# thawro/pytorch-human-pose

Hardware: AMD Instinct MI355X
Metric: images/sec (fwd+decode) HigherHRNet-W32 512px (higher is better)
Workload: dtype bf16; 1 GPU; HigherHRNet-W32 inference bf16, batch 32 @ 512x512 per GPU (conv fwd on N(0,1) images + AE decode on constructed maps, 10 people/image, det_thr 0.05, tag_thr 0.5, adjust+refine); global_batch=32, parallelism=image-sharded replicas x1, no data-path collective

## Files before the change

### include/hhrnet.h

```cpp
#ifndef HHRNET_H
#define HHRNET_H
#include <stdint.h>

#ifdef __cplusplus
extern "C" {
#endif

#define HH_ABI_VERSION 3
#define HH_DTYPE_BF16 1
#define HH_DTYPE_FP8 2
#define HH_DTYPE_F16 3

typedef struct hh_net hh_net;
typedef struct hh_decoder hh_decoder;

int hh_abi_version(void);
const char *hh_last_error(void);

hh_net *hh_create(int num_kpts, int C, int dtype);
void hh_destroy(hh_net *net);

hh_net *hh_create_classifier(int C, int num_classes, int dtype);
int hh_forward_classifier(hh_net *net, const float *images, int B, int H, int W, float *logits, void *stream);

int hh_num_params(const hh_net *net);
const char *hh_param_name(const hh_net *net, int index);
int hh_param_shape(const hh_net *net, int index, int64_t shape[4]);

int hh_load_weights(hh_net *net, const char *name, const float *host, const int64_t *shape, int ndim);
int hh_finalize(hh_net *net);

int hh_calibrate(hh_net *net, const float *images, int B, int H, int W, int rounds, void *stream);

int hh_e4m3_encode(const float *x, int64_t n, unsigned char *out);
int hh_e4m3_decode(const unsigned char *x, int64_t n, float *out);

int hh_reserve(hh_net *net, int B, int H, int W);
int64_t hh_workspace_bytes(const hh_net *net);

int hh_forward(hh_net *net, const float *images, int B, int H, int W, float *init_heatmaps, float *deconv_heatmaps,
               int use_graph, void *stream);

int hh_set_multi_lane(hh_net *net, int enable);

int hh_debug_check_plan(const hh_net *net);

double hh_forward_flops(const hh_net *net, int B, int H, int W);

int hh_profile_enable(hh_net *net, int enable);
int hh_profile_count(const hh_net *net);
int hh_profile_get(hh_net *net, int index, int *cfg, double *flops, double *bytes, float *ms, float *kernel_ms, const char **layer);
int hh_profile_clock(hh_net *net, int index, double *ghz);
int hh_conv_config(int cfg, int out[7]);
int hh_conv_config_double_buffered(int cfg);

int hh_debug_conv_bench(int cfg, int B, int Hin, int Win, int cin, int cout, int with_res, int relu, int iters,
                        float *ms_per_launch, unsigned long long *stamps16, int ref_cfg, float *max_diff);

int hh_debug_bb_bench(int B, int H, int W, int iters, float *ms_per_launch, unsigned long long *stamps64);
int hh_debug_bb_compare(int B, int H, int W, int iters, float *max_diff, float *ms_classic, float *ms_pc);

int hh_debug_bb_cover(int B, int H, int W, int tall, int num_cus, int64_t counts[4]);

int hh_set_taps(hh_net *net, int enable);
int hh_num_taps(const hh_net *net);
const char *hh_tap_name(const hh_net *net, int index);
int hh_tap_shape(const hh_net *net, int index, int64_t shape[4]);
int hh_tap_read(hh_net *net, int index, float *host_nchw);

int hh_preprocess_u8(const unsigned char *image_hwc, int h, int w, const double dst_to_src[6], float *out_nchw, int H, int W,
                     const float mean[3], const float stdv[3], void *stream);

typedef struct hh_image_desc {
    long long offset;
    int h, w;
    double dst_to_src[6];
} hh_image_desc;
int hh_preprocess_u8_batch(const unsigned char *images_base, const hh_image_desc *descs_dev, int n, float *out_nchw, int H, int W,
                           const float mean[3], const float stdv[3], void *stream);

int hh_flip_images(const float *images, float *out, int B, int C, int H, int W, void *stream);
int hh_flip_merge(float *hm, int64_t hm_bstride, const float *hm_flipped, int64_t hmf_bstride, const float *tags_flipped,
                  int64_t tf_bstride, float *tags_out, int64_t to_bstride, const int32_t *perm_host, int B, int K,
                  int h, int w, void *stream);

hh_decoder *hh_decoder_create(int num_kpts, int max_people, double det_thr, double tag_thr);
void hh_decoder_destroy(hh_decoder *dec);
int hh_decoder_reserve(hh_decoder *dec, int B, int H, int W, int E);
int hh_decoder_set_exact_topk(hh_decoder *dec, int enable);

#define HH_DECODE_FALLBACK 1
#define HH_DECODE_SOLVER_GUARD 2
int hh_decode(hh_decoder *dec, const float *hm_q, int64_t hm_q_bstride, const float *hm_h, int64_t hm_h_bstride,
              const float *const *tags_q, const int64_t *tags_bstride, int E, int B, int hq, int wq, int adjust,
              int refine, float *joints, float *scores, int32_t *num_people, int32_t *flags, void *stream);

int hh_parse(hh_decoder *dec, const float *hm_full, const float *tags_full, int E, int B, int H, int W, int adjust,
             int refine, float *joints, float *scores, int32_t *num_people, int32_t *flags, void *stream);
// ... 309 lines not shown
```

### pytorch-human-pose_amd/csrc/capi.cpp

```cpp
#include <cmath>
#include <cstdint>
#include <cstring>
#include <string>
#include <vector>

#include "../../include/hhrnet.h"
#include "engine.h"
#include "optim_math.h"
#include "grad_stats_math.h"
#include "ema_math.h"
#include "render_math.h"
#include "panel_math.h"
#include "coco_eval_math.h"
#include "crowd_mask_math.h"
#include "track_math.h"

const char *hh_get_error();
int hh_tap_read_impl(hh_net *n, int index, float *host);

extern "C" {

int hh_abi_version(void) { return HH_ABI_VERSION; }
const char *hh_last_error(void) { return hh_get_error(); }

// ... 70 lines not shown
int hh_e4m3_encode(const float *x, int64_t n, unsigned char *out)
{
    for (int64_t i = 0; i < n; ++i) out[i] = hh_f32_to_e4m3(x[i]);
    return 0;
}
int hh_e4m3_decode(const unsigned char *x, int64_t n, float *out)
{
    for (int64_t i = 0; i < n; ++i) out[i] = hh_e4m3_to_f32(x[i]);
    return 0;
}
int hh_finalize(hh_net *net) { return net->finalize(); }
int hh_calibrate(hh_net *net, const float *images, int B, int H, int W, int rounds, void *stream)
{
    if (!images || B <= 0 || H <= 0 || W <= 0 || H % 32 || W % 32) { hh_set_error("hh_calibrate: need images [B,3,H,W] with H, W multiples of 32"); return 1; }
    return net->calibrate(images, B, H, W, rounds > 0 ? rounds : 2, (hipStream_t)stream);
}
int hh_reserve(hh_net *net, int B, int H, int W) { return net->reserve(B, H, W); }
int64_t hh_workspace_bytes(const hh_net *net) { return net->ws_bytes; }

int hh_forward(hh_net *net, const float *images, int B, int H, int W, float *init_heatmaps, float *deconv_heatmaps,
               int use_graph, void *stream)
{
    if (net->kind != 0) { hh_set_error("hh_forward: classifier handle, use hh_forward_classifier"); return 1; }
    if (!images || !init_heatmaps || !deconv_heatmaps) { hh_set_error("hh_forward: null buffer"); return 1; }
    if (B <= 0 || H <= 0 || W <= 0 || H % 32 || W % 32) { hh_set_error("hh_forward: H and W must be positive multiples of 32"); return 1; }
    return net->forward(images, B, H, W, init_heatmaps, deconv_heatmaps, use_graph, (hipStream_t)stream);
}
double hh_forward_flops(const hh_net *net, int B, int H, int W) { return net->flops(B, H, W); }

int hh_set_multi_lane(hh_net *net, int enable)
{
    net->multi_lane = enable != 0;
    for (auto &g : net->graphs) hipGraphExecDestroy(g.exec);
    net->graphs.clear();
    return 0;
}
int hh_set_taps(hh_net *net, int enable) { net->taps_enabled = enable != 0; return 0; }
int hh_num_taps(const hh_net *net) { return (int)net->taps.size(); }
const char *hh_tap_name(const hh_net *net, int i) { return (i >= 0 && i < (int)net->taps.size()) ? net->taps[i].name.c_str() : nullptr; }
int hh_tap_shape(const hh_net *net, int i, int64_t shape[4])
{
    if (i < 0 || i >= (int)net->taps.size()) return 1;
    const TensorDesc &d = net->tensors[net->taps[i].tensor];
    shape[0] = net->lastB; shape[1] = net->taps[i].C; shape[2] = net->lastH >> d.shift; shape[3] = net->lastW >> d.shift;
    return 0;
}
int hh_tap_read(hh_net *net, int index, float *host_nchw) { return hh_tap_read_impl(net, index, host_nchw); }

int hh_debug_check_plan(const hh_net *net)
{
    std::string why;
    if (net->check_plan(&why)) { hh_set_error("schedule hazard: " + why); return 1; }
    return 0;
}

int hh_profile_enable(hh_net *net, int enable) { net->prof_enabled = enable != 0; net->prof_clk = enable == 2; net->prof_used = 0; return 0; }
int hh_profile_count(const hh_net *net) { return (int)net->prof_used; }
int hh_profile_get(hh_net *net, int i, int *cfg, double *flops, double *bytes, float *ms, float *kernel_ms, const char **layer)
{
    if (i < 0 || i >= (int)net->prof_used) { hh_set_error("hh_profile_get: index out of range"); return 1; }
    const ProfRecord &r = net->prof[i];
    HH_CHECK_HIP(hipEventSynchronize(r.e1));
    HH_CHECK_HIP(hipEventElapsedTime(ms, r.e0, r.e1));
    *cfg = r.cfg; *flops = r.flops; *bytes = r.bytes;
    *layer = net->layers[net->ops[r.op].layer].conv.c_str();
    *kernel_ms = -1.f;
    if (r.slot >= 0 && net->prof_clk && net->d_clk && net->clk_khz > 0) {
        unsigned long long t[2];
        HH_CHECK_HIP(hipMemcpy(t, net->d_clk + 4 * r.slot, 16, hipMemcpyDeviceToHost));
        if (t[1] > t[0]) *kernel_ms = (float)((double)(t[1] - t[0]) / net->clk_khz);
    }
    return 0;
}
int hh_profile_clock(hh_net *net, int i, double *ghz)
{
    if (i < 0 || i >= (int)net->prof_used) { hh_set_error("hh_profile_clock: index out of range"); return 1; }
    const ProfRecord &r = net->prof[i];
    *ghz = 0.0;
    if (r.slot >= 0 && net->prof_clk && net->d_clk && net->clk_khz > 0) {
        unsigned long long t[2];
        HH_CHECK_HIP(hipEventSynchronize(r.e1));
        HH_CHECK_HIP(hipMemcpy(t, net->d_clk + 4 * r.slot + 2, 16, hipMemcpyDeviceToHost));
        if (t[1]) *ghz = (double)t[0] / (double)t[1] * net->clk_khz * 1e-6;
    }
    return 0;
}
int hh_conv_config(int cfg, int out[7])
{
    if (cfg >= 1000 && cfg - 1000 < conv_fp8_num_configs()) {
        const Fp8ConvConfig &c = conv_fp8_config(cfg - 1000);
        out[0] = c.KS; out[1] = c.S; out[2] = c.KC; out[3] = c.NT; out[4] = 1; out[5] = c.PT; out[6] = c.TW;
        return 0;
    }
    if (cfg < 0 || cfg >= conv_num_configs()) return 1;
    const ConvConfig &c = conv_config(cfg);
    out[0] = c.KS; out[1] = c.S; out[2] = c.KC; out[3] = c.NT; out[4] = c.WC; out[5] = c.PT; out[6] = c.TW;
    return 0;
}

int hh_conv_config_double_buffered(int cfg)
{
    if (cfg >= 1000 && cfg - 1000 < conv_fp8_num_configs()) return 0;
    if (cfg < 0 || cfg >= conv_num_configs()) return -1;
    return conv_config(cfg).DB;
}

// ... 1562 lines not shown
```

### pytorch-human-pose_amd/csrc/engine.cpp

```cpp
#include "engine.h"
#include "f16_host.h"

#include <cmath>
#include <cstdlib>
#include <cstring>

static thread_local std::string g_err;
LaunchProbe &hh_launch_probe()
{
    static thread_local LaunchProbe p;
    return p;
}
void hh_set_error(const std::string &msg) { g_err = msg; }
const char *hh_get_error() { return g_err.c_str(); }

PlanSwitches PlanSwitches::from_env()
{
    auto on = [](const char *name) { const char *v = getenv(name); return v && *v && strcmp(v, "0"); };
    auto is = [](const char *name, const char *val) { const char *v = getenv(name); return v && !strcmp(v, val); };
    PlanSwitches s;
    s.bb32_tile = is("HH_BB32", "tile");
    s.no_bb64 = on("HH_NO_BB64");
    s.no_stem_fused = on("HH_NO_STEM_FUSED");
    s.no_junc_pair = on("HH_NO_JUNC_PAIR");
    s.full_join = on("HH_FULL_JOIN");
    s.no_fusion_merge = on("HH_NO_FUSION_MERGE");
    s.no_fused_upsum = on("HH_NO_FUSED_UPSUM");
    s.poison_ws = on("HH_POISON_WS");
    s.poison_lds = on("HH_POISON_LDS");
    s.no_head_fold = on("HH_NO_HEAD_FOLD");
    s.no_conv_db = on("HH_NO_CONV_DB");
    s.no_final_fuse = on("HH_NO_FINAL_FUSE");
    s.keep_waits = on("HH_KEEP_WAITS");
    s.event_system_fence = on("HH_EVENT_SYSTEM_FENCE");
    s.bb_tall = on("HH_NO_BB_TALL") ? 0 : is("HH_BB_TALL", "always") ? 2 : 1;
    s.fp8_trunk8 = is("HH_FP8_TRUNK", "e4m3");
    s.fp8_heads8 = is("HH_FP8_HEADS", "e4m3");
    return s;
}

static inline int round_up(int v, int m) { return (v + m - 1) / m * m; }

static inline bf16_raw f2bf(float f)
{
    uint32_t u;
    memcpy(&u, &f, 4);
    if ((u & 0x7fffffffu) > 0x7f800000u) return (bf16_raw)((u >> 16) | 0x40);
    u += 0x7fffu + ((u >> 16) & 1u);
    return (bf16_raw)(u >> 16);
}
static inline float bf2f(bf16_raw h)
{
    uint32_t u = (uint32_t)h << 16;
    float f;
    memcpy(&f, &u, 4);
    return f;
}
bf16_raw hh_net::cvt16(float f) const { return act() ? hh_f32_to_f16(f) : f2bf(f); }
float hh_net::widen16(bf16_raw v) const { return act() ? hh_f16_to_f32(v) : bf2f(v); }
int hh_net::check_packed(const std::vector<bf16_raw> &packed, const std::string &param_name) const
{
    if (!act()) return 0;
    for (bf16_raw v : packed)
        if (hh_f16_is_inf(v)) {
            hh_set_error("hh_finalize: " + param_name + ": a BatchNorm-folded weight exceeds the fp16 range (+-65504); use a bf16 handle for this checkpoint");
            return 1;
        }
    return 0;
}

int hh_net::add_param(const std::string &name, std::vector<int64_t> shape, bool counter)
{
    ParamSlot p;
    p.name = name;
    p.shape = std::move(shape);
// ... 114 lines not shown
                p_conv(up + ".conv2", mid, mid, 3); p_bn(up + ".bn2", mid);
                p_conv(up + ".conv3", mid, outs[i], 1); p_bn(up + ".bn3", outs[i]);
                if (w[i] != outs[i]) { p_conv(up + ".downsample.0", w[i], outs[i], 1); p_bn(up + ".downsample.1", outs[i]); }
            }
            for (int i = 0; i < 3; ++i) {
                const std::string dpn = hp + ".downsample_blocks." + std::to_string(i);
                p_conv(dpn + ".0", outs[i], outs[i + 1], 3, true); p_bn(dpn + ".1", outs[i + 1]);
            }
            p_conv(hp + ".final_conv.0", 1024, 2048, 1, true); p_bn(hp + ".final_conv.1", 2048);
            n.add_param(hp + ".classifier.weight", {n.num_classes, 2048});
            n.add_param(hp + ".classifier.bias", {n.num_classes});
            return;
        }
        p_conv("init_heatmaps_head", C, 2 * K, 1, true);
        const std::string dp = "deconv_layers.0";
        n.add_param(dp + ".deconv.0.weight", {C + 2 * K, C, 4, 4});
        p_bn(dp + ".deconv.1", C);
        for (int r = 0; r < 4; ++r) {
            const std::string rp = dp + ".resid_blocks." + std::to_string(r);
            p_conv(rp + ".conv1", C, C, 3); p_bn(rp + ".bn1", C);
            p_conv(rp + ".conv2", C, C, 3); p_bn(rp + ".bn2", C);
        }
        p_conv(dp + ".final_layer", C, K, 1, true);
    }

    int T(int C, int shift, bool zero = false)
    {
        TensorDesc t;
        t.C = C; t.shift = shift; t.zero_init = zero;
        n.tensors.push_back(t);
        return (int)n.tensors.size() - 1;
    }
    int L(const std::string &conv, const std::string &bn, int cin, int cout, int ks, int stride, const std::string &bias = "")
    {
        ConvLayer l;
        l.conv = conv; l.bn = bn; l.bias = bias; l.cin = cin; l.cout = cout; l.ks = ks; l.stride = stride;
        n.layers.push_back(l);
        return (int)n.layers.size() - 1;
    }
    Op &conv(int layer, int in, int out, int relu, int res = -1)
    {
        Op o;
        o.kind = OP_CONV; o.layer = layer; o.in = in; o.out = out; o.relu = relu; o.res = res; o.lane = lane;
        n.ops.push_back(o);
        return n.ops.back();
    }
    Op &cb(const std::string &p, const char *c, const char *b, int cin, int cout, int ks, int stride, int in, int out,
           int relu, int res = -1)
    {
        return conv(L(p + "." + c, p + "." + b, cin, cout, ks, stride), in, out, relu, res);
    }
    void basic_blocks(const std::string &prefix, int C, int x, int m, int nscales = 0, int branch = 0)
    {
        for (int u = 0; u < 4; ++u) {
            const std::string up = prefix + "." + std::to_string(u);
            const bool fused_fp8 = n.dtype == 2 && bb_fp8_supported(C) && branch == 0;
            if (((C == 32 || (C == 64 && !n.sw.no_bb64)) && n.is16()) || fused_fp8) {
                Op o;
                o.kind = OP_BB;
                o.layer = L(up + ".conv1", up + ".bn1", C, C, 3, 1);
                o.layer2 = L(up + ".conv2", up + ".bn2", C, C, 3, 1);
                o.in = (u & 1) ? m : x;
                o.out = (u & 1) ? x : m;
                o.lane = lane;
                o.siblings = nscales > 1;
                n.ops.push_back(o);
            } else {
                cb(up, "conv1", "bn1", C, C, 3, 1, x, m, 1);
                cb(up, "conv2", "bn2", C, C, 3, 1, m, x, 1, x);
            }
        }
    }
    void tap(const std::string &name, int tensor, int C, int coff = 0)
    {
        TapInfo t;
        t.name = name; t.tensor = tensor; t.coff = coff; t.C = C;
        n.taps.push_back(t);
        Op o;
        o.kind = OP_TAP; o.tap = (int)n.taps.size() - 1; o.lane = lane;
        n.ops.push_back(o);
    }

    void build_plan()
    {
        const int C = n.C, K = n.K;
        const int w[4] = {C, 2 * C, 4 * C, 8 * C};
        const std::string bb = "backbone";
        const bool stem_fused = n.is16() && !n.sw.no_stem_fused;
        const int S1 = stem_fused ? -1 : T(64, 1), X = T(64, 2);
        {
            Op o;
            o.kind = OP_STEM; o.layer = L(bb + ".conv1", bb + ".bn1", 3, 64, 3, 2); o.out = stem_fused ? X : S1;
            n.layers[o.layer].stem = true;
            if (stem_fused) {
                o.layer2 = L(bb + ".conv2", bb + ".bn2", 64, 64, 3, 2);
                n.layers[o.layer2].stem2 = true;
            }
            n.ops.push_back(o);
        }
        if (!stem_fused) conv(L(bb + ".conv2", bb + ".bn2", 64, 64, 3, 2), S1, X, 1);

        const bool jpair = n.is16() && !n.sw.no_junc_pair;
        const int t1 = T(64, 2), t2 = T(64, 2), t2b = jpair ? T(64, 2) : t2, Y = T(256, 2);
        auto unit = [&](int u) { return bb + ".stages.0.blocks.0.scales_blocks.0." + std::to_string(u); };
        cb(unit(0), "conv1", "bn1", 64, 64, 1, 1, X, t1, 1);
        const int DS = n.dtype == 2 ? T(256, 2) : -1;
        int prev_conv3 = -1, ds_layer = -1;
        for (int u = 0; u < 4; ++u) {
            const std::string up = unit(u);
            const int t2u = (u & 1) ? t2b : t2, t2p = (u & 1) ? t2 : t2b;
// ... 283 lines not shown
                        for (int j = 0; j < 8; ++j, ++o) {
                            const int co = cg * COUT_T + ci_o, ci = ch * KC + c8 * 8 + j;
                            if (co >= cout || ci >= cin) continue;
                            float v;
                            if (transposed) v = W[(((size_t)ci * cout + co) * 4 + ky) * 4 + kx];
                            else v = W[(((size_t)co * cin + ci) * ks + ky) * ks + kx];
                            packed[o] = act_dtype ? hh_f32_to_f16(v * scale[co]) : f2bf(v * scale[co]);
                        }
            }
}

int hh_family_pick(int ks, int stride, int cin_pad, int coutp, int *KC, int *NT)
{
    if (ks == 3 && stride == 1) *KC = (cin_pad % 32 == 0) ? 32 : 16;
    else if (ks == 1) *KC = (cin_pad % 32 == 0) ? 32 : 16;
    else *KC = 16;
    *NT = (coutp % 64 == 0) ? 2 : 1;
    for (int i = 0; i < conv_num_configs(); ++i) {
        const ConvConfig &c = conv_config(i);
        if (c.KS == ks && c.S == stride && c.KC == *KC && c.NT == *NT && !c.DB) return 0;
    }
    return 1;
}

float hh_net::bn_fold(const std::string &bn, int co, const float *cb, float *shift) const
{
    const float g = param(bn + ".weight")[co], bta = param(bn + ".bias")[co];
    const float mu = param(bn + ".running_mean")[co], var = param(bn + ".running_var")[co];
    const float sc = g / std::sqrt(var + 1e-5f);
    *shift = cb ? bta + (*cb - mu) * sc : bta - mu * sc;
    return sc;
}

void hh_net::fold_layer(const ConvLayer &l, int coutp, std::vector<float> &scale, std::vector<float> &shift) const
{
    scale.assign(coutp, 0.f);
    shift.assign(coutp, 0.f);
    for (int co = 0; co < l.cout; ++co) {
        const float cb = l.bias.empty() ? 0.f : param(l.bias)[co];
        if (l.bn.empty()) { scale[co] = 1.f; shift[co] = cb; }
        else scale[co] = bn_fold(l.bn, co, &cb, &shift[co]);
    }
}

int hh_net::finalize()
{
    for (auto &p : params)
        if (!p.loaded && !p.counter) { hh_set_error("hh_finalize: parameter never loaded: " + p.name); return 1; }
    HH_CHECK_HIP(conv_init());
    HH_CHECK_HIP(bb_fused_init());
    HH_CHECK_HIP(stem_fused_init());
    HH_CHECK_HIP(bbpc_init());
    HH_CHECK_HIP(bb64_fused_init());
    HH_CHECK_HIP(junction_init());
    if (dtype == 2 && kind != 0) { hh_set_error("hh_finalize: the fp8 path covers HigherHRNet only"); return 1; }
    {
        int dev = 0;
        hipDeviceProp_t prop;
        HH_CHECK_HIP(hipGetDevice(&dev));
        HH_CHECK_HIP(hipGetDeviceProperties(&prop, dev));
        num_cus = prop.multiProcessorCount;
    }
    for (auto &l : layers) {
        if (l.stem) {
            const std::vector<float> &W = param(l.conv + ".weight");
            std::vector<bf16_raw> packed(64 * 32, 0);
            std::vector<float> shift(64);
            for (int co = 0; co < 64; ++co) {
                const float sc = bn_fold(l.bn, co, nullptr, &shift[co]);
                for (int t = 0; t < 27; ++t) {
                    const int kk = t / 16, hh = (t % 16) / 8, j = t % 8;
                    packed[((((co / 32) * 2 + kk) * 2 + hh) * 32 + co % 32) * 8 + j] = cvt16(W[(size_t)co * 27 + t] * sc);
                }
            }
            if (check_packed(packed, l.conv + ".weight")) return 1;
            if (hh_upload(&l.d_w, packed.data(), packed.size() * 2) || hh_upload(&l.d_bias, shift.data(), 64 * 4)) return 1;
            continue;
        }
        if (dtype == 2 && !l.hi) continue;
        const int cin_pad0 = round_up(l.cin, 16), coutp = round_up(l.cout, 32);
        if (l.stem2) { l.KC = 64; l.NT = 2; }
        else if (hh_family_pick(l.ks, l.stride, cin_pad0, coutp, &l.KC, &l.NT)) {
            hh_set_error("no kernel family for conv " + l.conv);
            return 1;
        }
        l.db = !sw.no_conv_db && !l.stem2 && l.ks == 3 && l.stride == 1 && !l.transposed && l.mconv.empty() && l.cin >= 128 &&
               l.cin % 16 == 0 && coutp % 64 == 0;
        if (l.db) { l.KC = 16; l.NT = 2; }
        l.cin_pad = round_up(l.cin, l.KC);
        const int COUT_T = 32 * l.NT;
        l.ncg = coutp / COUT_T;
        if (!l.mconv.empty()) {
            std::vector<float> Wm((size_t)l.cout * l.cin * 9, 0.f), one(coutp, 1.f), shift(coutp, 0.f);
            int c0 = 0;
            for (size_t m = 0; m < l.mconv.size(); ++m) {
                if (l.mcin[m] % l.KC) { hh_set_error("merged fusion conv: input width not a multiple of the chunk size"); return 1; }
                const std::vector<float> &Wj = param(l.mconv[m] + ".weight");
                for (int co = 0; co < l.cout; ++co) {
                    float sh;
                    const float sc = bn_fold(l.mbn[m], co, nullptr, &sh);
                    shift[co] += sh;
                    for (int ci = 0; ci < l.mcin[m]; ++ci)
                        for (int t = 0; t < 9; ++t) Wm[((size_t)co * l.cin + c0 + ci) * 9 + t] = Wj[((size_t)co * l.mcin[m] + ci) * 9 + t] * sc;
                    if (act())
                        for (int i = 0; i < l.mcin[m] * 9; ++i)
                            if (hh_f16_is_inf(hh_f32_to_f16(Wj[(size_t)co * l.mcin[m] * 9 + i] * sc))) return check_packed({0x7c00}, l.mconv[m] + ".weight");
// ... 360 lines not shown
    p.nsrc = op.nup;
    for (int j = 0; j < op.nup; ++j) {
        const ConvLayer &l = layers[op.up_layer[j]];
        const TensorDesc &t = tensors[op.up[j]];
        if (t.shift != b0.shift + j + 1 || l.KC != 32 || l.NT != 1 || l.ncg != 1 || l.cin != (op.C << (j + 1))) {
            hh_set_error("plan: fusion output 0 does not fit fusion_up.hip (HH_NO_FUSED_UPSUM=1)");
            return 1;
        }
        p.src[j] = t.ptr; p.src_cs[j] = t.C; p.w[j] = l.d_w; p.bias[j] = l.d_bias;
    }
    p.out = o.ptr; p.out_cs = o.C;
    p.B = B; p.H = H >> b0.shift; p.W = W >> b0.shift;
    if (prof_enabled && prof_record(op, HH_CFG_FUSION_UP, op_cost(op, B, H, W), &p.clk)) return 1;
    HH_CHECK_HIP(fusion_up_launch(p, s, act()));
    return 0;
}

int hh_net::enqueue_junc(const Op &op, int B, int H, int W, hipStream_t s)
{
    const ConvLayer &l3 = layers[op.layer];
    JuncParams p{};
    const TensorDesc &ti = tensors[op.in];
    p.t2 = tensors[op.in].ptr; p.t2_cs = tensors[op.in].C;
    if (op.res >= 0) { p.res = tensors[op.res].ptr; p.res_cs = tensors[op.res].C; }
    if (op.in2 >= 0) { p.x = tensors[op.in2].ptr; p.x_cs = tensors[op.in2].C; p.wd = layers[op.layer2].d_w; p.bd = layers[op.layer2].d_bias; }
    p.w3 = l3.d_w; p.b3 = l3.d_bias;
    if (op.layer4 >= 0) {
        p.t2a = tensors[op.in3].ptr; p.t2a_cs = tensors[op.in3].C;
        p.w3a = layers[op.layer4].d_w; p.b3a = layers[op.layer4].d_bias;
    }
    if (op.layer3 >= 0) { p.w1 = layers[op.layer3].d_w; p.b1 = layers[op.layer3].d_bias; p.t1 = tensors[op.out2].ptr; p.t1_cs = tensors[op.out2].C; }
    if (op.out >= 0) { p.y = tensors[op.out].ptr; p.y_cs = tensors[op.out].C; }
    p.npix = B * (H >> ti.shift) * (W >> ti.shift);
    if (prof_enabled && prof_record(op, HH_CFG_JUNCTION, op_cost(op, B, H, W), &p.clk)) return 1;
    HH_CHECK_HIP(junction_launch(p, num_cus, s, act()));
    return 0;
}

int hh_net::enqueue_bb(const Op &op, int B, int H, int W, float *o2, bool multi, hipStream_t s, int *fin_done)
{
    const ConvLayer &l1 = layers[op.layer], &l2 = layers[op.layer2];
    const TensorDesc &ti = tensors[op.in], &to = tensors[op.out];
    BBParams p{};
    p.in = ti.ptr; p.in_cs = ti.C; p.out = to.ptr; p.out_cs = to.C;
    p.w1 = l1.d_w; p.w2 = l2.d_w; p.b1 = l1.d_bias; p.b2 = l2.d_bias;
    p.B = B; p.H = H >> ti.shift; p.W = W >> ti.shift;
    p.tall = sw.bb_tall;
    if (op.fin >= 0 && !sw.no_final_fuse && !sw.bb32_tile && !taps_enabled && o2) {
        const ConvLayer &lf = layers[ops[op.fin].layer];
        p.fin_w = lf.d_wfin; p.fin_b = lf.d_bias; p.fin_out = o2; p.fin_K = lf.cout;
        if (lf.d_wfin && bbpc_final_supported(p)) *fin_done = op.fin;
        else { p.fin_w = nullptr; p.fin_b = nullptr; p.fin_out = nullptr; p.fin_K = 0; }
    }
    const int cfg = l1.cout == 64 ? HH_CFG_BB64_FUSED : HH_CFG_BB_FUSED;
    if (prof_enabled && prof_record(op, cfg, op_cost(op, B, H, W, p.fin_out != nullptr), &p.clk)) return 1;
    const int fat = multi && op.siblings ? (num_cus + 1) / 2 : num_cus;
    if (l1.cout == 64) HH_CHECK_HIP(bb64_fused_launch(p, fat, s, act()));
    else if (!sw.bb32_tile && bbpc_supported(p)) HH_CHECK_HIP(bbpc_launch(p, fat, s, act()));
    else if (act()) { hh_set_error("hh_forward: the tile-form 32-channel block (tensors of 2 GB and more) has no fp16 form"); return 1; }
    else HH_CHECK_HIP(bb_fused_launch(p, num_cus, s));
    return 0;
}

int hh_net::enqueue_conv(const Op &op, int B, int H, int W, float *o1, float *o2, hipStream_t s)
{
    const ConvLayer &l = layers[op.layer];
    const TensorDesc &ti = tensors[op.in];
    ConvParams p{};
    hh_conv_geometry(p, l, op, B, H >> ti.shift, W >> ti.shift, o1, o2);
    p.in = dtype == 2 ? ti.ptr16 : ti.ptr; p.in_cs = ti.C; p.in_coff = op.in_coff;
    p.w = l.d_w; p.bias = l.d_bias;
    if (op.out >= 0) {
        const TensorDesc &to = tensors[op.out];
        p.out = dtype == 2 ? to.ptr16 : to.ptr; p.out_cs = to.C; p.out_coff = op.out_coff;
    }
    if (op.res >= 0) {
        const TensorDesc &tr = tensors[op.res];
        p.res = dtype == 2 ? tr.ptr16 : tr.ptr; p.res_cs = tr.C; p.res_coff = op.res_coff;
    }
    if (op.in2 >= 0) {
        const TensorDesc &t2 = tensors[op.in2];
        if (t2.C != ti.C || t2.shift != ti.shift || (op.in3 >= 0 && (tensors[op.in3].C != ti.C || tensors[op.in3].shift != ti.shift))) {
            hh_set_error("merged fusion conv: inputs differ in shape or pixel stride");
            return 1;
        }
        p.nch0 = l.mcin[0] / l.KC;
        p.nch1 = l.mcin[1] / l.KC;
        p.src_delta1 = t2.ptr - (ti.ptr + op.in_coff);
        if (op.in3 >= 0) p.src_delta2 = tensors[op.in3].ptr - (ti.ptr + op.in_coff);
    }
    p.cout_store = op.cout_store >= 0 ? op.cout_store : round_up(l.cout, 8);
    const int cfg = hh_pick_config(l.ks, l.stride, l.KC, l.NT, p.Wo, l.db);
    const ConvConfig &c = conv_config(cfg);
    p.tiles_x = (p.Wo + c.TW - 1) / c.TW;
    p.tiles_y = (p.Ho + c.th() - 1) / c.th();
    if (prof_enabled && prof_record(op, cfg, op_cost(op, B, H, W), &p.clk)) return 1;
    HH_CHECK_HIP(conv_launch(cfg, p, s, act()));
    return 0;
}

int hh_net::forward(const float *images, int B, int H, int W, float *o1, float *o2, int use_graph, hipStream_t s)
{
    if (!finalized) { hh_set_error("hh_forward: call hh_finalize first"); return 1; }
    if (dtype == 2 && !calibrated) { hh_set_error("hh_forward: fp8 handle without activation scales, call hh_calibrate first"); return 1; }
    if (B > rB || H > rH || W > rW || !ws_ready || (taps_enabled && !taps.empty() && !taps[0].copy))
        if (reserve(B, H, W)) return 1;
    lastB = B; lastH = H; lastW = W;
    if (!use_graph || s == nullptr || taps_enabled || prof_enabled || sw.poison_lds || multi_lane)
        return enqueue(images, B, H, W, o1, o2, s);
    for (auto &g : graphs)
// ... 206 lines not shown
```

### pytorch-human-pose_amd/csrc/engine.h

```cpp
#pragma once
#include <map>
#include <string>
#include <vector>

#include "kernels.h"

void hh_set_error(const std::string &msg);
void hh_pack_weights(const float *W, const float *scale, int ks, int cin, int cout, int KC, int COUT_T, bool transposed,
                     int py, int px, std::vector<unsigned short> &packed, int act_dtype = 0);
#define HH_CHECK_HIP(expr)                                                                             \
    do {                                                                                               \
        hipError_t _e = (expr);                                                                        \
        if (_e != hipSuccess) {                                                                        \
            hh_set_error(std::string(#expr) + ": " + hipGetErrorString(_e));                           \
            return 1;                                                                                  \
        }                                                                                              \
    } while (0)

struct ParamSlot {
    std::string name;
    std::vector<int64_t> shape;
    std::vector<float> data;
    bool loaded = false;
    bool counter = false;
// ... 39 lines not shown
    int layer = -1, layer2 = -1;
    int layer3 = -1;
    int layer4 = -1;
    int in2 = -1, out2 = -1;
    int in3 = -1;
    int in = -1, in_coff = 0;
    int out = -1, out_coff = 0;
    int res = -1, res_coff = 0;
    int relu = 0;
    int f32_out = 0;
    int cout_store = -1;
    int scatter = 0;
    int up[3] = {-1, -1, -1}, up_shift[3] = {0, 0, 0}, nup = 0;
    int up_layer[3] = {-1, -1, -1};
    int C = 0;
    int tap = -1;
    bool res8 = false;
    int fin = -1;
    bool siblings = false;
    bool hi = false;
    int lane = 0;
    int nlanes = 0;
    int dep_from = 0;
    float s_in = 1.f, s_in2 = 1.f, s_res = 1.f, s_out = 1.f, s_up[3] = {1.f, 1.f, 1.f};
    float s_mid = 1.f;
    int amax_slot = -1;
};

struct TapInfo {
    std::string name;
    int tensor, coff, C;
    bf16_raw *copy = nullptr;
    float scale = 1.f;
    bool is16 = false;
};

struct ProfRecord {
    int op, cfg;
    double flops, bytes;
    hipEvent_t e0, e1;
    int slot;
};

struct GraphEntry {
    const void *images;
    void *o1, *o2;
    int B, H, W;
    hipGraphExec_t exec;
};

struct PlanSwitches {
    bool bb32_tile = false;
    bool no_bb64 = false;
    bool no_stem_fused = false;
    bool no_junc_pair = false;
    bool full_join = false;
    bool no_fusion_merge = false;
    bool no_fused_upsum = false;
    bool event_system_fence = false;
    bool keep_waits = false;
    bool no_final_fuse = false;
    int bb_tall = 1;
    bool no_conv_db = false;
    bool no_head_fold = false;
    bool fp8_trunk8 = false;
    bool fp8_heads8 = false;
    bool poison_ws = false;
    bool poison_lds = false;
    static PlanSwitches from_env();
};

struct OpCost { double flops = 0, bytes = 0; };

struct hh_net {
    int K, C, dtype;
    int kind = 0;
    int num_classes = 0;
    float *d_pool = nullptr, *d_fc_w = nullptr, *d_fc_b = nullptr;
    int pool_cap = 0;
    std::vector<ParamSlot> params;
    std::map<std::string, int> param_index;
    std::vector<ConvLayer> layers;
    std::vector<TensorDesc> tensors;
    std::vector<Op> ops;
    std::vector<TapInfo> taps;
    bool taps_enabled = false;
    bool finalized = false;
    int num_cus = 256;
    int rB = 0, rH = 0, rW = 0;
    int lastB = 0, lastH = 0, lastW = 0;
    int64_t ws_bytes = 0;
    bool ws_ready = false;
    std::vector<void *> allocs;
    std::vector<GraphEntry> graphs;
    bool prof_enabled = false;
    bool prof_clk = false;
    std::vector<ProfRecord> prof;
    size_t prof_used = 0;
    unsigned long long *d_clk = nullptr;
    double clk_khz = 0;
    hipStream_t lane_streams[4] = {nullptr, nullptr, nullptr, nullptr};
    int lane_priority = 0;
    bool lane_priority_set = false;
    std::vector<hipEvent_t> lane_events;
    size_t lane_events_used = 0;
    bool multi_lane = true;
// ... 77 lines not shown
```

### pytorch-human-pose_amd/csrc/kernels.h

```cpp
#pragma once
#include <hip/hip_runtime.h>
#include <stdint.h>

#include <hip/hip_ext.h>

typedef uint16_t bf16_raw;

struct LaunchProbe { hipEvent_t start = nullptr, stop = nullptr; };
LaunchProbe &hh_launch_probe();
#define HH_LAUNCH(kernel, grid, block, lds, stream, ...)                                                            \
    do {                                                                                                            \
        LaunchProbe &lp_ = hh_launch_probe();                                                                       \
        if (lp_.start) {                                                                                            \
            hipExtLaunchKernelGGL(kernel, grid, block, lds, stream, lp_.start, lp_.stop, 0, __VA_ARGS__);           \
            lp_ = LaunchProbe{};                                                                                    \
        } else {                                                                                                    \
            hipLaunchKernelGGL(kernel, grid, block, lds, stream, __VA_ARGS__);                                      \
        }                                                                                                           \
    } while (0)

struct ConvParams {
    const bf16_raw *in;
    int in_cs, in_coff;
    int Hin, Win;
// ... 104 lines not shown
struct BBParams {
    const bf16_raw *in; int in_cs;
    bf16_raw *out; int out_cs;
    const bf16_raw *w1, *w2;
    const float *b1, *b2;
    int B, H, W;
    int tiles_x, tiles_y, ntiles;
    int tall;
    int VH;
    bf16_raw *trash;
    const bf16_raw *fin_w;
    const float *fin_b;
    float *fin_out;
    int fin_K;
    unsigned long long *stamps;
    unsigned long long *clk;
};
constexpr int BBPC_TH = 14, BBPC_TW = 32;
struct BBGeom { int b, oy0, ox0; };
__host__ __device__ inline int bbpc_band(int i, int ntiles, unsigned grid)
{
    return ((ntiles & 7) == 0 && (grid & 7) == 0) ? (i & 7) * (ntiles >> 3) + (i >> 3) : i;
}
__host__ __device__ __forceinline__ BBGeom bbpc_geom(int tb, int tiles_x, int tiles_per_img, int VH)
{
    const int u = tb / tiles_per_img, tt = tb % tiles_per_img;
    const int oy = (tt / tiles_x) * BBPC_TH, bq = oy / VH;
    return BBGeom{u + bq, oy - bq * VH, (tt % tiles_x) * BBPC_TW};
}
__host__ __device__ __forceinline__ int bbpc_rowmap(int b, int y, int B, int H, int VH)
{
    const bool wrap = y >= VH;
    const int ya = wrap ? y - VH : y, bb = wrap ? b + 1 : b;
    return (((unsigned)ya < (unsigned)H) & (bb < B)) ? bb * H + ya : -1;
}
__host__ __device__ inline bool bbpc_patch_wrap(int yy, int VH) { return yy >= VH; }
__host__ __device__ inline bool bbpc_patch_row(int yy, bool wrap, bool next, int H, int VH)
{
    return ((unsigned)(wrap ? yy - VH : yy) < (unsigned)H) & (!wrap | next);
}
bool bbpc_cover(int B, int H, int W, int tall, int num_cus, long long counts[4]);

#define HH_PROF_SLOTS 1024
#define HH_CFG_BB_FUSED 100
hipError_t bb_fused_init();
hipError_t bb_fused_launch(BBParams p, int num_cus, hipStream_t s);
hipError_t bbpc_init();
bool bbpc_supported(const BBParams &p);
bool bbpc_final_supported(const BBParams &p);
hipError_t bbpc_launch(BBParams p, int num_cus, hipStream_t s, int act_dtype = 0);
#define HH_CFG_BB64_FUSED 103
hipError_t bb64_fused_init();
hipError_t bb64_fused_launch(BBParams p, int num_cus, hipStream_t s, int act_dtype = 0);

struct JuncParams {
    const bf16_raw *t2; int t2_cs;
    const bf16_raw *res; int res_cs;
    const bf16_raw *x; int x_cs;
    const bf16_raw *t2a; int t2a_cs;
    const bf16_raw *w3a; const float *b3a;
    const bf16_raw *w3, *wd, *w1;
    const float *b3, *bd, *b1;
    bf16_raw *y; int y_cs;
    bf16_raw *t1; int t1_cs;
    int npix;
    unsigned long long *clk;
};
#define HH_CFG_JUNCTION 101
hipError_t junction_init();
hipError_t junction_launch(const JuncParams &p, int num_cus, hipStream_t s, int act_dtype = 0);

struct StemParams {
    const float *images;
    const bf16_raw *w;
    const float *bias;
    bf16_raw *out; int out_cs;
    int B, H, W;
    unsigned long long *clk;
    unsigned char *out_fp8;
    float out_inv_scale;
    unsigned *absmax;
};
#define HH_CFG_STEM 102
hipError_t stem_conv_launch(const StemParams &p, hipStream_t s);
struct StemFusedParams {
    const float *images;
    const bf16_raw *w1;
    const float *b1;
    const bf16_raw *w2;
    const float *b2;
    bf16_raw *out; int out_cs;
    int B, H, W;
    unsigned long long *clk;
};
#define HH_CFG_STEM_FUSED 106
hipError_t stem_fused_init();
bool stem_fused_supported(const StemFusedParams &p);
hipError_t stem_fused_launch(const StemFusedParams &p, int num_cus, hipStream_t s, int act_dtype = 0);


struct UpAddParams {
    const bf16_raw *base; int base_cs, base_coff;
    const bf16_raw *up[3]; int up_cs[3]; int up_shift[3]; int nup;
    bf16_raw *out; int out_cs, out_coff;
    int B, H, W, C, relu;
};
// ... 174 lines not shown
```

Baseline: 7153 images/sec.

## Fuse 128/256-channel basic blocks into a single wide MFMA kernel

Adds a fused basic-block kernel for 128- and 256-channel branches that computes conv1 into an LDS halo tile and then conv2 plus residual in the same workgroup. Weights and input patches are double-buffered across channel chunks. It is enabled by default for C=128 (256 stays off), replacing two separate conv launches and the round trip of the intermediate activation through global memory. The cost is recomputing the halo region, heavy register pressure, and a bounded occupancy of two workgroups per CU.

```diff
diff --git a/include/hhrnet.h b/include/hhrnet.h
--- a/include/hhrnet.h
+++ b/include/hhrnet.h
@@ -44,6 +44,8 @@
 int hh_set_multi_lane(hh_net *net, int enable);
 
 int hh_debug_check_plan(const hh_net *net);
+
+int hh_debug_launch_count(const hh_net *net);
 
 double hh_forward_flops(const hh_net *net, int B, int H, int W);
 
diff --git a/pytorch-human-pose_amd/csrc/basicblock_fused_wide.hip b/pytorch-human-pose_amd/csrc/basicblock_fused_wide.hip
--- /dev/null
+++ b/pytorch-human-pose_amd/csrc/basicblock_fused_wide.hip
@@ -0,0 +1,300 @@
+#include "mfma_dev.h"
+
+namespace {
+template <int C> struct WideGeom;
+template <> struct WideGeom<128> { static constexpr int TH = 8, TW = 16; };
+template <> struct WideGeom<256> { static constexpr int TH = 4, TW = 8; };
+
+template <bool KXMAJOR> struct StepOrder {
+    static constexpr int ky(int st) { return KXMAJOR ? st % 3 : st / 3; }
+    static constexpr int kx(int st) { return KXMAJOR ? st / 3 : st % 3; }
+};
+
+template <int C>
+constexpr size_t wide_lds_bytes()
+{
+    using G = WideGeom<C>;
+    constexpr int MPIX = (G::TH + 2) * (G::TW + 2), MT = (MPIX + 31) / 32;
+    return 2 * (size_t)(G::TH + 4) * (G::TW + 4) * 48 + (size_t)MT * 32 * (C * 2 + 16);
+}
+static_assert(wide_lds_bytes<128>() <= 80 * 1024 && wide_lds_bytes<256>() <= 80 * 1024, "two workgroups per CU");
+}
+
+template <typename E, int C, bool KXMAJOR>
+__global__ __launch_bounds__(256, 2) void bb_wide_kernel(const BBParams p)
+{
+    using G = WideGeom<C>;
+    using SO = StepOrder<KXMAJOR>;
+    constexpr int TH = G::TH, TW = G::TW, MW = TW + 2, IH = TH + 4, IW = TW + 4;
+    constexpr int NCH = C / 16, NT = C / 128, RPT = 32 / TW;
+    constexpr int MPIX = (TH + 2) * MW, MT = (MPIX + 31) / 32, OT = TH * TW / 32;
+    constexpr int PSP = 48, PSM = C * 2 + 16;
+    constexpr int PATCH_BYTES = IH * IW * PSP, P_UNITS = IH * IW * 2, NPL = (P_UNITS + 255) / 256;
+    static_assert(NPL <= 9 && OT * 32 == TH * TW && NT * 4 * 32 == C, "tile geometry");
+
+    extern __shared__ __attribute__((aligned(16))) char smem[];
+    char *lds_m = smem + 2 * PATCH_BYTES;
+
+    const int tid = threadIdx.x;
+    if (p.clk && tid == 0 && blockIdx.x < 256) atomicMin(p.clk, wall_clock64());
+    const int wave = tid >> 6, lane = tid & 63;
+    const int r = lane & 31, h = lane >> 5;
+
+    int t = blockIdx.x;
+    if ((p.ntiles & 7) == 0) t = (t & 7) * (p.ntiles >> 3) + (t >> 3);
+    const int tx = t % p.tiles_x, ty = (t / p.tiles_x) % p.tiles_y, b = t / (p.tiles_x * p.tiles_y);
+    const int oy0 = ty * TH, ox0 = tx * TW;
+    const bf16_raw *in_b = p.in + (size_t)b * p.H * p.W * p.in_cs;
+
+    const bf16_raw *psrc[NPL];
+    unsigned pmask = 0;
+#pragma unroll
+    for (int i = 0; i < NPL; ++i) {
+        const int u = tid + 256 * i, pix = u >> 1, part = u & 1;
+        const int iy = oy0 - 2 + pix / IW, ix = ox0 - 2 + pix % IW;
+        const bool ok = u < P_UNITS && (unsigned)iy < (unsigned)p.H && (unsigned)ix < (unsigned)p.W;
+        psrc[i] = ok ? in_b + ((size_t)iy * p.W + ix) * p.in_cs + part * 8 : in_b;
+        pmask |= ok ? (1u << i) : 0u;
+    }
+    u32x4 preg[NPL];
+    auto patch_load = [&](auto ic, int c) {
+        constexpr int i = decltype(ic)::value;
+        preg[i] = *reinterpret_cast<const u32x4 *>(psrc[i] + c * 16);
+    };
+    auto patch_write = [&](int buf) {
+        static_for<NPL>([&](auto ic) {
+            constexpr int i = decltype(ic)::value;
+            const int u = tid + 256 * i;
+            if (u < P_UNITS)
+                *reinterpret_cast<u32x4 *>(smem + buf * PATCH_BYTES + (u >> 1) * PSP + (u & 1) * 16) = (pmask >> i) & 1u ? preg[i] : u32x4{0u, 0u, 0u, 0u};
+        });
+    };
+
+    const u32x4 *wq[2][NT];
+#pragma unroll
+    for (int nt = 0; nt < NT; ++nt) {
+        const int ct = wave * NT + nt;
+        const size_t off = (size_t)(ct >> 1) * NCH * (9 * 128) + h * 64 + (ct & 1) * 32 + r;
+        wq[0][nt] = reinterpret_cast<const u32x4 *>(p.w1) + off;
+        wq[1][nt] = reinterpret_cast<const u32x4 *>(p.w2) + off;
+    }
+    u32x4 wa[2][9][NT];
+    auto w_load = [&](auto setc, auto stc, const u32x4 *const *wsrc) {
+        constexpr int set = decltype(setc)::value, st = decltype(stc)::value;
+        constexpr int tap = SO::ky(st) * 3 + SO::kx(st);
+#pragma unroll
+        for (int nt = 0; nt < NT; ++nt) wa[set][st][nt] = wsrc[nt][tap * 128];
+    };
+
+    int paddr[MT];
+#pragma unroll
+    for (int q = 0; q < MT; ++q) {
+        const int pidx = q * 32 + r, pc = pidx < MPIX ? pidx : MPIX - 1;
+        paddr[q] = ((pc / MW) * IW + pc % MW) * PSP + h * 16;
+    }
+
+    static_for<NPL>([&](auto ic) { patch_load(ic, 0); });
+    static_for<9>([&](auto stc) { w_load(std::integral_constant<int, 0>{}, stc, wq[0]); });
+
+    f32x16 acc1[MT][NT];
+#pragma unroll
+    for (int nt = 0; nt < NT; ++nt)
+#pragma unroll
+        for (int g = 0; g < 4; ++g) {
+            const float4 bv = *reinterpret_cast<const float4 *>(p.b1 + (wave * NT + nt) * 32 + 8 * g + 4 * h);
+#pragma unroll
+            for (int q = 0; q < MT; ++q) {
+                acc1[q][nt][4 * g + 0] = bv.x + 0.f; acc1[q][nt][4 * g + 1] = bv.y + 0.f;
+                acc1[q][nt][4 * g + 2] = bv.z + 0.f; acc1[q][nt][4 * g + 3] = bv.w + 0.f;
+            }
+        }
+    patch_write(0);
+    lds_barrier();
+
+    auto conv1_chunk = [&](auto parc, int c) {
+        constexpr int par = decltype(parc)::value;
+        const char *pb = smem + par * PATCH_BYTES;
+        const bool last = c + 1 == NCH;
+        const int cn = last ? c : c + 1;
+        const u32x4 *wn[NT];
+#pragma unroll
+        for (int nt = 0; nt < NT; ++nt) wn[nt] = last ? wq[1][nt] : wq[0][nt] + cn * (9 * 128);
+        u32x4 fb[2][MT];
+        auto ldb = [&](int st, int buf) {
+            const int off = (SO::ky(st) * IW + SO::kx(st)) * PSP;
+#pragma unroll
+            for (int q = 0; q < MT; ++q) fb[buf][q] = *reinterpret_cast<const u32x4 *>(pb + paddr[q] + off);
+        };
+        ldb(0, 0);
+        __builtin_amdgcn_sched_group_barrier(0x100, MT, 0);
+        static_for<9>([&](auto stc) {
+            constexpr int st = decltype(stc)::value;
+            if constexpr (st + 1 < 9) {
+                ldb(st + 1, (st + 1) & 1);
+                __builtin_amdgcn_sched_group_barrier(0x100, MT, 0);
+            }
+            constexpr int npl = st < NPL ? 1 : 0;
+            if constexpr (npl) patch_load(stc, cn);
+            w_load(std::integral_constant<int, 1 - par>{}, stc, wn);
+            __builtin_amdgcn_sched_group_barrier(0x020, NT + npl, 0);
+#pragma unroll
+            for (int q = 0; q < MT; ++q)
+#pragma unroll
+                for (int nt = 0; nt < NT; ++nt) acc1[q][nt] = E::mfma(wa[par][st][nt], fb[st & 1][q], acc1[q][nt]);
+            __builtin_amdgcn_sched_group_barrier(0x8, MT * NT, 0);
+        });
+        patch_write(1 - par);
+        lds_barrier();
+    };
+#pragma unroll 1
+    for (int c = 0; c < NCH; c += 2) {
+        conv1_chunk(std::integral_constant<int, 0>{}, c);
+        conv1_chunk(std::integral_constant<int, 1>{}, c + 1);
+    }
+
+    int opix[OT];
+    unsigned ovalid = 0;
+    u32x4 rv[OT][NT][2];
+#pragma unroll
+    for (int q = 0; q < OT; ++q) {
+        const int oy = oy0 + q * RPT + r / TW, ox = ox0 + r % TW;
+        const bool valid = oy < p.H && ox < p.W;
+        opix[q] = valid ? oy * p.W + ox : 0;
+        ovalid |= valid ? (1u << q) : 0u;
+#pragma unroll
+        for (int nt = 0; nt < NT; ++nt)
+#pragma unroll
+            for (int m = 0; m < 2; ++m) {
+                const int c0 = (wave * NT + nt) * 32 + 16 * m + 8 * h;
+                const u32x4 v = *reinterpret_cast<const u32x4 *>(in_b + (size_t)opix[q] * p.in_cs + c0);
+                rv[q][nt][m] = valid ? v : u32x4{0u, 0u, 0u, 0u};
+            }
+    }
+#pragma unroll
+    for (int q = 0; q < MT; ++q) {
+        const int pidx = q * 32 + r;
+        const int gy = oy0 - 1 + pidx / MW, gx = ox0 - 1 + pidx % MW;
+        const bool outside = ((unsigned)gy >= (unsigned)p.H) | ((unsigned)gx >= (unsigned)p.W);
+#pragma unroll
+        for (int nt = 0; nt < NT; ++nt) {
+            u32x4 o[2];
+            pack_rows16<E>(acc1[q][nt], o);
+            char *dst = lds_m + pidx * PSM + (wave * NT + nt) * 64 + h * 16;
+            *reinterpret_cast<u32x4 *>(dst) = outside ? u32x4{0u, 0u, 0u, 0u} : o[0];
+            *reinterpret_cast<u32x4 *>(dst + 32) = outside ? u32x4{0u, 0u, 0u, 0u} : o[1];
+        }
+    }
+    f32x16 acc2[OT][NT];
+#pragma unroll
+    for (int nt = 0; nt < NT; ++nt) {
+        float4 bs[4];
+#pragma unroll
+        for (int g = 0; g < 4; ++g) bs[g] = *reinterpret_cast<const float4 *>(p.b2 + (wave * NT + nt) * 32 + 8 * g + 4 * h);
+#pragma unroll
+        for (int q = 0; q < OT; ++q)
+#pragma unroll
+            for (int m = 0; m < 2; ++m) {
+                auto s0 = __builtin_amdgcn_permlane32_swap(rv[q][nt][m][0], rv[q][nt][m][2], false, false);
+                auto s1 = __builtin_amdgcn_permlane32_swap(rv[q][nt][m][1], rv[q][nt][m][3], false, false);
+                const unsigned x0 = s0[0], y0 = s0[1], x1 = s1[0], y1 = s1[1];
+                const float4 ba = bs[2 * m], bb = bs[2 * m + 1];
+                acc2[q][nt][8 * m + 0] = ba.x + E::lo(x0); acc2[q][nt][8 * m + 1] = ba.y + E::hi(x0);
+                acc2[q][nt][8 * m + 2] = ba.z + E::lo(x1); acc2[q][nt][8 * m + 3] = ba.w + E::hi(x1);
+                acc2[q][nt][8 * m + 4] = bb.x + E::lo(y0); acc2[q][nt][8 * m + 5] = bb.y + E::hi(y0);
+                acc2[q][nt][8 * m + 6] = bb.z + E::lo(y1); acc2[q][nt][8 * m + 7] = bb.w + E::hi(y1);
+            }
+    }
+    lds_barrier();
+
+    const int maddr = ((r / TW) * MW + r % TW) * PSM + h * 16;
+    auto conv2_chunk = [&](auto parc, int c) {
+        constexpr int par = decltype(parc)::value;
+        const int cn = c + 1 == NCH ? c : c + 1;
+        const u32x4 *wn[NT];
+#pragma unroll
+        for (int nt = 0; nt < NT; ++nt) wn[nt] = wq[1][nt] + cn * (9 * 128);
+        const char *mb = lds_m + maddr + c * 32;
+        u32x4 fb[2][OT];
+        auto ldb = [&](int st, int buf) {
+            const int off = (SO::ky(st) * MW + SO::kx(st)) * PSM;
+#pragma unroll
+            for (int q = 0; q < OT; ++q) fb[buf][q] = *reinterpret_cast<const u32x4 *>(mb + q * RPT * MW * PSM + off);
+        };
+        ldb(0, 0);
+        __builtin_amdgcn_sched_group_barrier(0x100, OT, 0);
+        static_for<9>([&](auto stc) {
+            constexpr int st = decltype(stc)::value;
+            if constexpr (st + 1 < 9) {
+                ldb(st + 1, (st + 1) & 1);
+                __builtin_amdgcn_sched_group_barrier(0x100, OT, 0);
+            }
+            w_load(std::integral_constant<int, 1 - par>{}, stc, wn);
+            __builtin_amdgcn_sched_group_barrier(0x020, NT, 0);
+#pragma unroll
+            for (int q = 0; q < OT; ++q)
+#pragma unroll
+                for (int nt = 0; nt < NT; ++nt) acc2[q][nt] = E::mfma(wa[par][st][nt], fb[st & 1][q], acc2[q][nt]);
+            __builtin_amdgcn_sched_group_barrier(0x8, OT * NT, 0);
+        });
+    };
+#pragma unroll 1
+    for (int c = 0; c < NCH; c += 2) {
+        conv2_chunk(std::integral_constant<int, 0>{}, c);
+        conv2_chunk(std::integral_constant<int, 1>{}, c + 1);
+    }
+
+    bf16_raw *out_b = p.out + (size_t)b * p.H * p.W * p.out_cs;
+#pragma unroll
+    for (int q = 0; q < OT; ++q)
+#pragma unroll
+        for (int nt = 0; nt < NT; ++nt) {
+            u32x4 o[2];
+            pack_rows16<E>(acc2[q][nt], o);
+            if ((ovalid >> q) & 1u) {
+                bf16_raw *dst = out_b + (size_t)opix[q] * p.out_cs + (wave * NT + nt) * 32 + 8 * h;
+                *reinterpret_cast<u32x4 *>(dst) = o[0];
+                *reinterpret_cast<u32x4 *>(dst + 16) = o[1];
+            }
+        }
+    if (p.clk && tid == 0 && blockIdx.x + 256 >= gridDim.x) atomicMax(p.clk + 1, wall_clock64());
+}
+
+namespace {
+typedef void (*bbw_fn)(const BBParams);
+template <int C>
+bbw_fn wide_fn(int act_dtype, bool kxmajor)
+{
+    if (act_dtype) return kxmajor ? bb_wide_kernel<ElemF16, C, true> : bb_wide_kernel<ElemF16, C, false>;
+    return kxmajor ? bb_wide_kernel<ElemBF16, C, true> : bb_wide_kernel<ElemBF16, C, false>;
+}
+bbw_fn wide_pick(int C, int act_dtype, bool kxmajor) { return C == 128 ? wide_fn<128>(act_dtype, kxmajor) : wide_fn<256>(act_dtype, kxmajor); }
+}
+
+bool bb_wide_supported(int C) { return C == 128 || C == 256; }
+size_t bb_wide_lds_bytes(int C) { return C == 128 ? wide_lds_bytes<128>() : wide_lds_bytes<256>(); }
+
+hipError_t bb_wide_init()
+{
+    for (int C : {128, 256})
+        for (int dt = 0; dt < 2; ++dt)
+            for (int kx = 0; kx < 2; ++kx) {
+                const hipError_t e = hipFuncSetAttribute(reinterpret_cast<const void *>(wide_pick(C, dt, kx != 0)), hipFuncAttributeMaxDynamicSharedMemorySize,
+                                                         (int)bb_wide_lds_bytes(C));
+                if (e != hipSuccess) return e;
+            }
+    return hipSuccess;
+}
+
+hipError_t bb_wide_launch(int C, BBParams p, hipStream_t s, int act_dtype)
+{
+    if (!bb_wide_supported(C) || (act_dtype != 0 && act_dtype != 1)) return hipErrorInvalidValue;
+    const int th = C == 128 ? WideGeom<128>::TH : WideGeom<256>::TH, tw = C == 128 ? WideGeom<128>::TW : WideGeom<256>::TW;
+    p.tiles_x = (p.W + tw - 1) / tw;
+    p.tiles_y = (p.H + th - 1) / th;
+    const long long ntiles = (long long)p.B * p.tiles_x * p.tiles_y;
+    if (ntiles > 0x7fffffffLL || (long long)p.H * p.W * (p.in_cs > p.out_cs ? p.in_cs : p.out_cs) > 0x7fffffffLL) return hipErrorInvalidValue;
+    p.ntiles = (int)ntiles;
+    const bool kxmajor = p.W > 16;
+    HH_LAUNCH(wide_pick(C, act_dtype, kxmajor), dim3((unsigned)p.ntiles), dim3(256), bb_wide_lds_bytes(C), s, p);
+    return hipGetLastError();
+}
diff --git a/pytorch-human-pose_amd/csrc/capi.cpp b/pytorch-human-pose_amd/csrc/capi.cpp
--- a/pytorch-human-pose_amd/csrc/capi.cpp
+++ b/pytorch-human-pose_amd/csrc/capi.cpp
@@ -146,6 +146,17 @@
     std::string why;
     if (net->check_plan(&why)) { hh_set_error("schedule hazard: " + why); return 1; }
     return 0;
+}
+
+int hh_debug_launch_count(const hh_net *net)
+{
+    int n = 0;
+    for (const Op &op : net->ops)
+        switch (op.kind) {
+        case OP_CONV: case OP_UPADD: case OP_BB: case OP_AVGPOOL: case OP_LINEAR: case OP_JUNC: case OP_STEM: case OP_QUANT: case OP_UPSUM: ++n; break;
+        default: break;
+        }
+    return n;
 }
 
 int hh_profile_enable(hh_net *net, int enable) { net->prof_enabled = enable != 0; net->prof_clk = enable == 2; net->prof_used = 0; return 0; }
diff --git a/pytorch-human-pose_amd/csrc/engine.cpp b/pytorch-human-pose_amd/csrc/engine.cpp
--- a/pytorch-human-pose_amd/csrc/engine.cpp
+++ b/pytorch-human-pose_amd/csrc/engine.cpp
@@ -21,6 +21,16 @@
     PlanSwitches s;
     s.bb32_tile = is("HH_BB32", "tile");
     s.no_bb64 = on("HH_NO_BB64");
+    {
+        const char *v = getenv("HH_BB_WIDE");
+        if (v && *v) { s.bb_wide128 = strstr(v, "128"); s.bb_wide256 = strstr(v, "256"); }
+        v = getenv("HH_NO_BB_WIDE");
+        if (v && *v && strcmp(v, "0")) {
+            const bool all = !strcmp(v, "1");
+            if (all || strstr(v, "128")) s.bb_wide128 = false;
+            if (all || strstr(v, "256")) s.bb_wide256 = false;
+        }
+    }
     s.no_stem_fused = on("HH_NO_STEM_FUSED");
     s.no_junc_pair = on("HH_NO_JUNC_PAIR");
     s.full_join = on("HH_FULL_JOIN");
@@ -241,10 +251,11 @@
     }
     void basic_blocks(const std::string &prefix, int C, int x, int m, int nscales = 0, int branch = 0)
     {
+        const bool wide = n.is16() && !n.sw.no_conv_db && ((C == 128 && n.sw.bb_wide128) || (C == 256 && n.sw.bb_wide256));
         for (int u = 0; u < 4; ++u) {
             const std::string up = prefix + "." + std::to_string(u);
             const bool fused_fp8 = n.dtype == 2 && bb_fp8_supported(C) && branch == 0;
-            if (((C == 32 || (C == 64 && !n.sw.no_bb64)) && n.is16()) || fused_fp8) {
+            if (((C == 32 || (C == 64 && !n.sw.no_bb64)) && n.is16()) || wide || fused_fp8) {
                 Op o;
                 o.kind = OP_BB;
                 o.layer = L(up + ".conv1", up + ".bn1", C, C, 3, 1);
@@ -634,6 +645,7 @@
     HH_CHECK_HIP(stem_fused_init());
     HH_CHECK_HIP(bbpc_init());
     HH_CHECK_HIP(bb64_fused_init());
+    HH_CHECK_HIP(bb_wide_init());
     HH_CHECK_HIP(junction_init());
     if (dtype == 2 && kind != 0) { hh_set_error("hh_finalize: the fp8 path covers HigherHRNet only"); return 1; }
     {
@@ -1100,10 +1112,13 @@
         if (lf.d_wfin && bbpc_final_supported(p)) *fin_done = op.fin;
         else { p.fin_w = nullptr; p.fin_b = nullptr; p.fin_out = nullptr; p.fin_K = 0; }
     }
-    const int cfg = l1.cout == 64 ? HH_CFG_BB64_FUSED : HH_CFG_BB_FUSED;
+    const bool wide = bb_wide_supported(l1.cout);
+    if (wide && !(l1.db && l2.db)) { hh_set_error("hh_forward: the wide fused block needs the KC = 16 weight image of its two convs"); return 1; }
+    const int cfg = wide ? HH_CFG_BB_WIDE : l1.cout == 64 ? HH_CFG_BB64_FUSED : HH_CFG_BB_FUSED;
     if (prof_enabled && prof_record(op, cfg, op_cost(op, B, H, W, p.fin_out != nullptr), &p.clk)) return 1;
     const int fat = multi && op.siblings ? (num_cus + 1) / 2 : num_cus;
-    if (l1.cout == 64) HH_CHECK_HIP(bb64_fused_launch(p, fat, s, act()));
+    if (wide) HH_CHECK_HIP(bb_wide_launch(l1.cout, p, s, act()));
+    else if (l1.cout == 64) HH_CHECK_HIP(bb64_fused_launch(p, fat, s, act()));
     else if (!sw.bb32_tile && bbpc_supported(p)) HH_CHECK_HIP(bbpc_launch(p, fat, s, act()));
     else if (act()) { hh_set_error("hh_forward: the tile-form 32-channel block (tensors of 2 GB and more) has no fp16 form"); return 1; }
     else HH_CHECK_HIP(bb_fused_launch(p, num_cus, s));
diff --git a/pytorch-human-pose_amd/csrc/engine.h b/pytorch-human-pose_amd/csrc/engine.h
--- a/pytorch-human-pose_amd/csrc/engine.h
+++ b/pytorch-human-pose_amd/csrc/engine.h
@@ -115,6 +115,8 @@
 struct PlanSwitches {
     bool bb32_tile = false;
     bool no_bb64 = false;
+    bool bb_wide128 = true;
+    bool bb_wide256 = false;
     bool no_stem_fused = false;
     bool no_junc_pair = false;
     bool full_join = false;
diff --git a/pytorch-human-pose_amd/csrc/kernels.h b/pytorch-human-pose_amd/csrc/kernels.h
--- a/pytorch-human-pose_amd/csrc/kernels.h
+++ b/pytorch-human-pose_amd/csrc/kernels.h
@@ -180,6 +180,11 @@
 #define HH_CFG_BB64_FUSED 103
 hipError_t bb64_fused_init();
 hipError_t bb64_fused_launch(BBParams p, int num_cus, hipStream_t s, int act_dtype = 0);
+#define HH_CFG_BB_WIDE 108
+bool bb_wide_supported(int C);
+size_t bb_wide_lds_bytes(int C);
+hipError_t bb_wide_init();
+hipError_t bb_wide_launch(int C, BBParams p, hipStream_t s, int act_dtype = 0);
 
 struct JuncParams {
     const bf16_raw *t2; int t2_cs;
```

New measurement: 7202 images/sec (median of 6 runs). No clear change (+0.7%).
